# david-wb/tiny-diffusion

Hardware: AMD Instinct MI355X
Metric: train images/s (q_sample+fwd+MSE+bwd+allreduce+Adam), MNIST 28x28 UNet fp32; 1000-step sample latency in `sample` (higher is better)
Workload: dtype f32; 1 GPU; diffusion.py unconditional MNIST 28x28 UNet, fp32, train step, batch 256/GPU (BASELINE.json configs[1]); global_batch=256, per_gpu_batch=256, parallelism=dp1

## Files before the change

### include/tdx.h

```cpp
#ifndef TDX_H
#define TDX_H

#include <stddef.h>
#include <stdint.h>

#ifdef __cplusplus
extern "C" {
#endif

#define TDX_VERSION 400

#define TDX_E_BADARG (-1)
#define TDX_E_SHAPE (-2)
#define TDX_E_WORKSPACE (-3)
#define TDX_E_STATE (-4)

typedef void* tdx_stream_t;

int tdx_version(void);
const char* tdx_error_string(int code);


int tdx_q_sample(const float* x0, const float* noise, const int64_t* t,
                 const float* sqrt_ac, const float* sqrt_1mac, float* x_t,
// ... 155 lines not shown
                           int B, int H, int W, int cin, int cout, int flags,
                           const float* in_scale, const float* in_shift,
                           const float* out_scale, const float* out_shift,
                           float* scratch, size_t scratch_floats, tdx_stream_t stream);
size_t tdx_conv3x3_splitk_scratch_floats(int B, int H, int W, int cin, int cout);
int tdx_conv3x3_wino_ok(int B, int H, int W, int cin, int cout);
int tdx_pack_conv3x3_wino(const float* w_oihw, float* u_fwd, float* u_dgrad, int cout, int cin, tdx_stream_t stream);
int tdx_conv3x3_fwd_wino(const float* in, const float* u, const float* bias, float* out, int B, int H, int W,
                         int cin, int cout, int flags, const float* out_scale, const float* out_shift,
                         float* stats_partial, tdx_stream_t stream);
int tdx_conv3x3_fwd_wino_infer(const float* in, const float* u, const float* bias, float* out, int B, int H, int W,
                               int cin, int cout, const float* out_scale, const float* out_shift, float* scratch,
                               size_t scratch_floats, tdx_stream_t stream);
int tdx_conv3x3_train_algo(int B, int H, int W, int cin, int cout, int role);
int tdx_conv3x3_infer_algo(int B, int H, int W, int cin, int cout);
int tdx_conv3x3_wgrad_wino_splits(int B, int H, int W, int cin, int cout);
int tdx_conv3x3_wgrad_wino(const float* in, const float* dy, float* dw_slabs, int B, int H, int W, int cin, int cout,
                           tdx_stream_t stream);
int tdx_conv3x3_wino_stat_tiles(int B, int H, int W);
int tdx_conv3x3_wino_stat_tile_rows(int B, int H, int W);
int tdx_pack_conv3x3_tiled(const float* w_oihw, float* w_tiled, int cout, int cin, tdx_stream_t stream);
int tdx_conv3x3_fwd_infer(const float* in, const float* w_tiled, const float* bias, float* out, int B, int H, int W,
                          int cin, int cout, const float* out_scale, const float* out_shift, float* scratch,
                          size_t scratch_floats, tdx_stream_t stream);
size_t tdx_conv3x3_infer_scratch_floats(int B, int H, int W, int cin, int cout);
int tdx_conv3x3_fwd_train(const float* in, const float* wpk, const float* bias, float* out, int B, int H, int W,
                          int cin, int cout, int flags, float* stats_partial, float* scratch,
                          size_t scratch_floats, tdx_stream_t stream);
size_t tdx_conv3x3_train_scratch_floats(int B, int H, int W, int cin, int cout);
int tdx_conv3x3_stat_tiles(int B, int H, int W, int cin, int cout);
// ... 44 lines not shown
                    const float* save_rstd, const float* gamma,
                    float* dgamma, float* dbeta, float* dbias, float* scratch,
                    int training, tdx_stream_t stream);
size_t tdx_bn_relu_bwd_scratch_floats(int64_t rows, int C);

int tdx_maxpool2_ceil_fwd(const float* y, const float* scale, const float* shift, float* out,
                          int B, int H, int W, int C, tdx_stream_t stream);
int tdx_maxpool2_ceil_bwd(const float* y, const float* scale, const float* shift,
                          const float* g_out, const float* skip_grad, float* g_in,
                          int B, int H, int W, int C, tdx_stream_t stream);

int tdx_bilinear_ac_fwd(const float* in, const float* scale, const float* shift,
                        const float* addend, float* out,
                        int B, int Hi, int Wi, int Ho, int Wo, int C,
                        int out_cstride, int out_coff, tdx_stream_t stream);
int tdx_bilinear_ac_bwd(const float* g_out, float* g_in,
                        int B, int Hi, int Wi, int Ho, int Wo, int C,
                        int g_cstride, int g_coff, tdx_stream_t stream);


enum {
  TDX_P_TE0_W = 0, TDX_P_TE0_B, TDX_P_TE2_W, TDX_P_TE2_B,
  TDX_P_CLASS_EMB,
  TDX_P_INIT_W, TDX_P_INIT_B,
  TDX_P_UNIT0,
  TDX_P_FINAL_W = TDX_P_UNIT0 + 13 * 4, TDX_P_FINAL_B,
  TDX_P_TP1_W, TDX_P_TP1_B, TDX_P_TP2_W, TDX_P_TP2_B, TDX_P_TP3_W, TDX_P_TP3_B,
  TDX_P_COUNT
};
#define TDX_B_COUNT (13 * 3)
// ... 60 lines not shown
typedef struct tdx_unet tdx_unet;

int tdx_unet_create(tdx_unet** out, int max_batch, int num_classes);
enum { TDX_UNET_MNIST = 0, TDX_UNET_LAION = 1, TDX_UNET_LATENT_MLP = 2 };
int tdx_unet_create_ex(tdx_unet** out, int max_batch, int kind, int num_classes);
int tdx_unet_create_hw(tdx_unet** out, int max_batch, int kind, int num_classes, int hw);
int tdx_unet_create_full(tdx_unet** out, int max_batch, int kind, int num_classes, int hw, int time_dim);
typedef int (*tdx_allreduce_fn)(void* user, double* device_buffer, int n, tdx_stream_t stream);
int tdx_unet_set_bn_sync(tdx_unet* u, tdx_allreduce_fn fn, void* user, double* buffer);

int tdx_unet_set_streams(tdx_unet* u, int mode);

#define TDX_PREC_F32 0
#define TDX_PREC_BF16 1
int tdx_unet_set_precision(tdx_unet* u, int precision);
int tdx_unet_destroy(tdx_unet* u);
size_t tdx_unet_workspace_bytes(const tdx_unet* u, int batch, int mode);

int tdx_unet_forward(tdx_unet* u, const void* const* params, void* const* buffers,
                     const float* x, const int64_t* t, const void* cond, float* out,
                     void* workspace, size_t workspace_bytes, int batch, int mode,
                     tdx_stream_t stream);

int tdx_unet_backward_stages(void);
int tdx_unet_backward(tdx_unet* u, const void* const* params, void* const* grads,
                      const float* d_out, void* workspace, size_t workspace_bytes,
                      int batch, int stage_lo, int stage_hi, tdx_stream_t stream);
int tdx_unet_backward_join(tdx_unet* u, tdx_stream_t stream);
int tdx_unet_backward_mark(tdx_unet* u, int slot);
int tdx_unet_backward_wait_mark(tdx_unet* u, int slot, tdx_stream_t stream);
// ... 61 lines not shown
```

### tiny_diffusion_amd/_lib.py

```python
from __future__ import annotations

import contextlib
import ctypes as C
import os

import torch

from . import _build

_c_float_p = C.c_void_p
_c_i64_p = C.c_void_p
_ptr = C.c_void_p


class TdxError(RuntimeError):
    pass


def _load():
    path = _build.LIB
    if not os.path.exists(path):
        if os.environ.get("TDX_NO_AUTOBUILD"):
            raise TdxError(
                f"{path} not found: build it with `python -m tiny_diffusion_amd._build` "
# ... 85 lines not shown
    "tdx_conv3x3_shape_ok": (C.c_int, [C.c_int] * 5),
    "tdx_conv3x3_tile_shape": (C.c_int, [C.c_int] * 6),
    "tdx_conv3x3_wgrad": (C.c_int, [_ptr, _ptr, _ptr, C.c_int, C.c_int, C.c_int, C.c_int, C.c_int,
                                    C.c_int, _ptr, _ptr, _ptr]),
    "tdx_conv3x3_wgrad_reduce": (C.c_int, [_ptr, _ptr, C.c_int, C.c_int, C.c_int, _ptr]),
    "tdx_bn_finalize": (C.c_int, [_ptr, C.c_int, C.c_int, C.c_int64, C.c_int, _ptr, _ptr, _ptr, _ptr, _ptr,
                                  _ptr, _ptr, _ptr, _ptr, C.c_int, _ptr]),
    "tdx_bn_relu_bwd": (C.c_int, [_ptr, _ptr, C.c_int64, C.c_int, _ptr, _ptr, _ptr, _ptr, _ptr,
                                  _ptr, _ptr, _ptr, _ptr, C.c_int, _ptr]),
    "tdx_bn_relu_bwd_scratch_floats": (C.c_size_t, [C.c_int64, C.c_int]),
    "tdx_maxpool2_ceil_fwd": (C.c_int, [_ptr, _ptr, _ptr, _ptr, C.c_int, C.c_int, C.c_int, C.c_int, _ptr]),
    "tdx_maxpool2_ceil_bwd": (C.c_int, [_ptr, _ptr, _ptr, _ptr, _ptr, _ptr, C.c_int, C.c_int, C.c_int,
                                        C.c_int, _ptr]),
    "tdx_bilinear_ac_fwd": (C.c_int, [_ptr, _ptr, _ptr, _ptr, _ptr, C.c_int, C.c_int, C.c_int, C.c_int,
                                      C.c_int, C.c_int, C.c_int, C.c_int, _ptr]),
    "tdx_bilinear_ac_bwd": (C.c_int, [_ptr, _ptr, C.c_int, C.c_int, C.c_int, C.c_int, C.c_int, C.c_int,
                                      C.c_int, C.c_int, _ptr]),
    "tdx_adam_step_dev": (C.c_int, [_ptr, _ptr, _ptr, _ptr, C.c_int64, _ptr, C.c_float, C.c_float, C.c_float, _ptr]),
    "tdx_step_begin": (C.c_int, [_ptr, _ptr, _ptr, C.c_int, _ptr]),
    "tdx_step_begin_sched": (C.c_int, [_ptr, _ptr, _ptr, _ptr, C.c_int, _ptr]),
    "tdx_p_sample_step_sched": (C.c_int, [_ptr, _ptr, _ptr, _ptr, _ptr, _ptr, _ptr, C.c_int64, _ptr]),
    "tdx_p_sample_step_sched_philox": (C.c_int, [_ptr, _ptr, _ptr, _ptr, _ptr, _ptr, C.c_int64, C.c_uint64, _ptr]),
    "tdx_linear_fwd": (C.c_int, [_ptr, C.c_int, _ptr, _ptr, _ptr, C.c_int, C.c_int, C.c_int, C.c_int, C.c_int, _ptr]),
    "tdx_linear_bwd": (C.c_int, [_ptr, C.c_int, _ptr, C.c_int, _ptr, _ptr, C.c_int, _ptr, _ptr, C.c_int, C.c_int,
                                 C.c_int, _ptr]),
    "tdx_linear_fwd_prec": (C.c_int, [_ptr, C.c_int, _ptr, _ptr, _ptr, C.c_int, C.c_int, C.c_int, C.c_int, C.c_int, C.c_int,
                                      _ptr]),
    "tdx_linear_bwd_prec": (C.c_int, [_ptr, C.c_int, _ptr, C.c_int, _ptr, _ptr, C.c_int, _ptr, _ptr, C.c_int, C.c_int,
                                      C.c_int, C.c_int, _ptr]),
    "tdx_vae_workspace_floats": (C.c_size_t, [C.c_int, C.c_int]),
# ... 12 lines not shown
    "tdx_act_fwd": (C.c_int, [_ptr, _ptr, C.c_int64, C.c_int, _ptr]),
    "tdx_act_bwd": (C.c_int, [_ptr, _ptr, _ptr, C.c_int64, C.c_int, _ptr]),
    "tdx_dropout": (C.c_int, [_ptr, _ptr, C.c_int64, C.c_int, C.c_float, C.c_uint64, C.c_uint64, _ptr]),
    "tdx_add": (C.c_int, [_ptr, _ptr, _ptr, C.c_int64, C.c_int64, _ptr]),
    "tdx_embedding_fwd": (C.c_int, [_ptr, _ptr, _ptr, C.c_int, C.c_int, _ptr]),
    "tdx_embedding_bwd": (C.c_int, [_ptr, _ptr, _ptr, C.c_int, C.c_int, C.c_int, _ptr]),
    "tdx_transformer_train_workspace_floats": (C.c_size_t, [_ptr]),
    "tdx_transformer_loss_grads": (C.c_int, [_ptr] * 8 + [C.c_int, C.c_uint64, C.c_uint64, _ptr, C.c_float] + [_ptr] * 4),
    "tdx_unet_create": (C.c_int, [C.POINTER(_ptr), C.c_int, C.c_int]),
    "tdx_unet_create_ex": (C.c_int, [C.POINTER(_ptr), C.c_int, C.c_int, C.c_int]),
    "tdx_unet_create_hw": (C.c_int, [C.POINTER(_ptr), C.c_int, C.c_int, C.c_int, C.c_int]),
    "tdx_unet_create_full": (C.c_int, [C.POINTER(_ptr), C.c_int, C.c_int, C.c_int, C.c_int, C.c_int]),
    "tdx_unet_set_bn_sync": (C.c_int, [_ptr, _ptr, _ptr, _ptr]),
    "tdx_unet_set_streams": (C.c_int, [_ptr, C.c_int]),
    "tdx_unet_set_precision": (C.c_int, [_ptr, C.c_int]),
    "tdx_pack_conv3x3_bf16": (C.c_int, [_ptr, _ptr, _ptr, C.c_int, C.c_int, _ptr]),
    "tdx_conv3x3_bf16_stat_tile_rows": (C.c_int, []),
    "tdx_conv3x3_fwd_bf16": (C.c_int, [_ptr, _ptr, _ptr, _ptr, C.c_int, C.c_int, C.c_int, C.c_int, C.c_int,
                                       C.c_int, _ptr, _ptr, _ptr, _ptr, _ptr, _ptr]),
    "tdx_conv3x3_wgrad_bf16": (C.c_int, [_ptr, _ptr, _ptr, C.c_int, C.c_int, C.c_int, C.c_int, C.c_int,
                                         C.c_int, _ptr, _ptr, _ptr]),
    "tdx_unet_destroy": (C.c_int, [_ptr]),
    "tdx_unet_workspace_bytes": (C.c_size_t, [_ptr, C.c_int, C.c_int]),
    "tdx_unet_forward": (C.c_int, [_ptr, _ptr, _ptr, _ptr, _ptr, _ptr, _ptr, _ptr, C.c_size_t, C.c_int,
                                   C.c_int, _ptr]),
    "tdx_unet_backward_stages": (C.c_int, []),
    "tdx_unet_backward": (C.c_int, [_ptr, _ptr, _ptr, _ptr, _ptr, C.c_size_t, C.c_int, C.c_int, C.c_int,
                                    _ptr]),
    "tdx_unet_backward_join": (C.c_int, [_ptr, _ptr]),
    "tdx_unet_backward_mark": (C.c_int, [_ptr, C.c_int]),
# ... 97 lines not shown
    return value.value


@contextlib.contextmanager
def tuned(**knobs):
    old = [(key, tune_get(key)) for key in knobs]
    try:
        for key, value in knobs.items():
            check(lib.tdx_tune_set(key.encode(), int(value)), f"tdx_tune_set({key})")
        yield
    finally:
        for key, value in reversed(old):
            check(lib.tdx_tune_set(key.encode(), value), f"tdx_tune_set({key})")


def ptr(t):
    return None if t is None else t.data_ptr()


def stream_ptr(device=None):
    return torch.cuda.current_stream(device).cuda_stream
```

### tiny_diffusion_amd/csrc/conv3x3.hip

```cpp
#include "internal.h"

#define BK 32
#define BKP 36

#include "conv_shared.h"

template <int BM, int BN, int EPI>
__global__ void __launch_bounds__(256)
conv3x3_igemm_kernel(ConvArgs a) {
  constexpr int WGM = 2, WGN = 2;
  constexpr int WTM = BM / WGM, WTN = BN / WGN;
  constexpr int TM = WTM / 32, TN = WTN / 32;
  constexpr int AI = BM / 32, BI = BN / 32;
  static_assert(TM >= 1 && TN >= 1, "wave tile must hold a 32x32 MFMA tile");

  extern __shared__ __attribute__((aligned(16))) float smem[];
  float* As = smem;
  float* Bs = smem + 2 * BM * BKP;

  const int tid = threadIdx.x;
  const int lane = tid & 63, wave = tid >> 6;
  const int l31 = lane & 31, half = lane >> 5;
  const int wm = wave / WGN, wn = wave % WGN;
  const int xb = blockIdx.x / (8 * a.tilesN), xr = blockIdx.x % (8 * a.tilesN);
// ... 1237 lines not shown
  a.bias = bias; a.out = scratch; a.out_scale = out_scale; a.out_shift = out_shift;
  a.B = B; a.H = H; a.W = W; a.Cin = cin; a.Cout = cout; a.M = (int)M;
  bool pooled = false;
  const int rc = splitk_finish<EPI_BNRELU>(a, out, scratch, splits, to_stream(stream), defer, pool ? pool->pooled : nullptr, &pooled);
  if (pool && !pooled) pool->pooled = nullptr;
  return rc;
}

extern "C" int tdx_conv3x3_fwd_wino_infer(const float* in, const float* u, const float* bias, float* out, int B, int H,
                                         int W, int cin, int cout, const float* out_scale, const float* out_shift,
                                         float* scratch, size_t scratch_floats, tdx_stream_t stream) {
  return tdx_conv3x3_fwd_wino_infer_ex(in, u, bias, out, B, H, W, cin, cout, out_scale, out_shift, scratch, scratch_floats,
                                       stream, nullptr, nullptr);
}

extern "C" int tdx_conv3x3_fwd_infer(const float* in, const float* w_tiled, const float* bias, float* out, int B, int H,
                                     int W, int cin, int cout, const float* out_scale, const float* out_shift,
                                     float* scratch, size_t scratch_floats, tdx_stream_t stream) {
  return tdx_conv3x3_fwd_infer_ex(in, w_tiled, bias, out, B, H, W, cin, cout, out_scale, out_shift, scratch,
                                  scratch_floats, stream, nullptr, nullptr);
}

extern "C" size_t tdx_conv3x3_infer_scratch_floats(int B, int H, int W, int cin, int cout) {
  int per;
  const int64_t M = (int64_t)B * H * W;
  if (B <= 0 || H <= 0 || W <= 0 || cin % BK || cout % 64) return 0;
  const int s = plan_infer(M, cin, cout, &per, (size_t)-1);
  return s > 1 ? (size_t)s * M * cout : 0;
}

// ... 578 lines not shown
```

### tiny_diffusion_amd/csrc/spatial.hip

```cpp
#include "internal.h"
#include "io16.h"

__device__ static inline float4 bnrelu4(float4 v, const float4& sc, const float4& sh) {
  v.x = fmaxf(fmaf(v.x, sc.x, sh.x), 0.f);
  v.y = fmaxf(fmaf(v.y, sc.y, sh.y), 0.f);
  v.z = fmaxf(fmaf(v.z, sc.z, sh.z), 0.f);
  v.w = fmaxf(fmaf(v.w, sc.w, sh.w), 0.f);
  return v;
}

struct BnBwdOps {
  const void* y;
  const float* scale; const float* shift; const float* mean; const float* rstd;
  float* partial;
};
__device__ static inline void bnbwd_acc(const float4& g, const float4& y, const float4& sc, const float4& sh,
                                        const float4& mu, const float4& rs, float4& s1, float4& s2) {
#define ACC(k)                                                  \
  {                                                             \
    const float gz = fmaf(y.k, sc.k, sh.k) > 0.f ? g.k : 0.f;   \
    s1.k += gz;                                                 \
    s2.k += gz * ((y.k - mu.k) * rs.k);                         \
  }
  ACC(x) ACC(y) ACC(z) ACC(w)
// ... 322 lines not shown
                             hipStream_t st, int io16) {
  const bool deferred = a_defer && a_defer->splits > 0;
  if ((!a && !deferred) || (!b && Cb) || !out || Ca % 4 || Cb % 4 || Ca <= 0 || Cb < 0) return TDX_E_BADARG;
  if (deferred && (!a_defer->partial || !a_defer->scale || !a_defer->shift)) return TDX_E_BADARG;
  ResizeSrc A{deferred ? static_cast<const void*>(a_defer->partial) : a, nullptr, Ha, Wa, Ca, ac_scale(Ha, Ho), ac_scale(Wa, Wo),
              deferred ? a_defer->splits : 0, deferred ? a_defer->slab : 0, deferred ? a_defer->bias : nullptr,
              deferred ? a_defer->scale : nullptr, deferred ? a_defer->shift : nullptr};
  ResizeSrc Bs{b, b_addend, Cb ? Hb : 1, Cb ? Wb : 1, Cb, Cb ? ac_scale(Hb, Ho) : 0.f, Cb ? ac_scale(Wb, Wo) : 0.f,
               0, 0, nullptr, nullptr, nullptr};
  const int64_t n = (int64_t)B * Ho * Wo * ((Ca + Cb) / 4);
  TDX_IO_DISPATCH(io16, T, bilinear_pair_fwd_kernel<T><<<ew_grid(n), 256, 0, st>>>(A, Bs, (T*)out, B, Ho, Wo));
  TDX_CHECK_LAUNCH();
  return 0;
}

#define BIL_MAXC 8
__device__ static inline void axis_adjoint(int i, float scale, int n_in, int n_out, int& lo,
                                           float (&w)[BIL_MAXC]) {
  int hi;
  if (scale > 0.f) {
    lo = max(0, (int)floorf((float)(i - 1) / scale) - 1);
    hi = min(n_out - 1, (int)ceilf((float)(i + 1) / scale) + 1);
  } else {
    lo = 0;
    hi = n_out - 1;
  }
  if (hi - lo + 1 > BIL_MAXC) hi = lo + BIL_MAXC - 1;
#pragma unroll
  for (int k = 0; k < BIL_MAXC; ++k) {
    const int o = lo + k;
// ... 226 lines not shown
```

### tiny_diffusion_amd/csrc/unet.hip

```cpp
#include "internal.h"
#include <algorithm>
#include <cstdlib>
#include <mutex>
#include <new>
#include <string>
#include <vector>

namespace {

struct UnitDef {
  int cin, cout, hw;
  int in_bn;
  int cin_real;
};

struct NetSpec {
  int in_ch, hw0, out_hw;
  int x0_ch, x0_real;
  int overlap;
  int time_dim;
  int enc_hw[4];
  int dec_hw[3];
  int skip_ch[3];
  UnitDef units[13];
// ... 30 lines not shown
  return true;
}


inline size_t align64(size_t n) { return (n + 63) / 64 * 64; }

struct Layout {
  size_t x, t, y;
  size_t sin, pre, emb, tp[3];
  size_t x0, Y[13], ss[13];
  size_t A[13];
  size_t ep[3], cat[3], d1a;
  size_t stats;
  size_t ksplit, ksplit_floats;
  size_t G1, G2, G3, G4, GS[3], gtp[3], slabs, slabs2, bnscr, smallp, smallp2, timescr;
  size_t gbuf;
  size_t total;
};

Layout make_layout(const NetSpec& S, int B) {
  Layout L;
  size_t o = 0;
  auto take = [&](size_t n) { size_t r = o; o += align64(n); return r; };
  const size_t b = (size_t)B;
  const size_t px0 = (size_t)S.hw0 * S.hw0;
  L.x = take(b * px0 * S.in_ch); L.t = take(2 * b); L.y = take(std::max<size_t>(2 * b, b * S.time_dim));
  L.sin = take(b * S.time_dim); L.pre = take(b * S.time_dim); L.emb = take(b * S.time_dim);
  for (int k = 0; k < 3; ++k) L.tp[k] = take(b * S.skip_ch[k]);
  L.x0 = take(b * px0 * S.x0_ch);
  size_t stats = 0, slabs = 0, bnscr = 0, gbuf = 0, ksplit = 0;
  for (int u = 0; u < 13; ++u) {
    const UnitDef& d = S.units[u];
    L.Y[u] = take(b * d.hw * d.hw * d.cout);
    L.ss[u] = take(4 * (size_t)d.cout);
    L.A[u] = (u + 1 < 13 && S.units[u + 1].in_bn) ? take(b * d.hw * d.hw * d.cout) : 0;
    stats = std::max(stats, (size_t)tdx_conv3x3_stat_tiles(B, d.hw, d.hw, d.cin, d.cout) * 2 * d.cout);
    slabs = std::max(slabs, (size_t)std::max(std::max(tdx_conv3x3_wgrad_splits(B, d.hw, d.hw, d.cin, d.cout),
                                                      tdx_conv3x3_wgrad_splits_bf16(B, d.hw, d.hw, d.cin, d.cout)),
                                             tdx_conv3x3_wgrad_wino_splits(B, d.hw, d.hw, d.cin, d.cout)) *
                                9 * (size_t)d.cin * d.cout);
    ksplit = std::max(ksplit, std::max(tdx_conv3x3_train_scratch_floats(B, d.hw, d.hw, d.cin, d.cout),
                                       tdx_conv3x3_train_scratch_floats(B, d.hw, d.hw, d.cout, d.cin)));
    bnscr = std::max(bnscr, tdx_bn_relu_bwd_scratch_floats((int64_t)b * d.hw * d.hw, d.cout));
    gbuf = std::max(gbuf, b * d.hw * d.hw * (size_t)std::max(d.cin, d.cout));
  }
  for (int k = 0; k < 3; ++k) {
    const int hp = S.enc_hw[k + 1];
    L.ep[k] = take(b * hp * hp * S.skip_ch[k]);
  }
  for (int k = 0; k < 3; ++k) {
    const UnitDef& d = S.units[7 + 2 * k];
    L.cat[k] = take(b * d.hw * d.hw * d.cin);
  }
  L.d1a = take(b * S.out_hw * S.out_hw * 64);
  gbuf = std::max(gbuf, b * (size_t)S.out_hw * S.out_hw * 64);
  L.stats = take(stats);
  L.ksplit_floats = ksplit;
  L.ksplit = take(ksplit);
  L.gbuf = gbuf;
  L.G1 = take(gbuf); L.G2 = take(gbuf); L.G3 = take(gbuf); L.G4 = take(gbuf);
  for (int k = 0; k < 3; ++k) {
    L.GS[k] = take(b * S.enc_hw[k] * S.enc_hw[k] * S.skip_ch[k]);
    L.gtp[k] = take(b * S.skip_ch[k]);
  }
  L.slabs = take(slabs);
  L.slabs2 = take(slabs);
  L.bnscr = take(bnscr);
  L.smallp = take((size_t)tdx_small_conv_wgrad_blocks(B, S.hw0, S.hw0) * tdx_small_conv_partial_width());
  L.smallp2 = take((size_t)tdx_small_conv_wgrad_blocks(B, S.hw0, S.hw0) * tdx_small_conv_partial_width());
  L.timescr = take(3 * b * S.time_dim);
  L.total = o;
  return L;
}

}

struct PlanHandles {
  hipStream_t side, side2, half;
  hipEvent_t ev[81];
};

// ... 181 lines not shown
extern "C" int tdx_unet_set_bn_sync(tdx_unet* u, tdx_allreduce_fn fn, void* user, double* buffer) {
  if (!u || (fn && !buffer)) return TDX_E_BADARG;
  if (!u->spec) return fn ? TDX_E_SHAPE : 0;
  u->bn_sync = fn;
  u->bn_sync_user = user;
  u->bn_sync_buf = buffer;
  return 0;
}

extern "C" int tdx_unet_set_streams(tdx_unet* u, int mode) {
  if (!u || mode < -1 || mode > 2) return TDX_E_BADARG;
  u->use_streams = mode < 0 ? (u->spec ? u->spec->overlap : 0) : mode;
  return 0;
}

extern "C" int tdx_unet_set_precision(tdx_unet* u, int precision) {
  if (!u || (precision != TDX_PREC_F32 && precision != TDX_PREC_BF16)) return TDX_E_BADARG;
  if (!u->spec) { u->precision = precision; return 0; }
  if (precision != u->precision) u->packed = false;
  u->precision = precision;
  u->io16 = precision == TDX_PREC_BF16 && g_knobs.bf16_storage ? 1 : 0;
  return 0;
}

extern "C" int tdx_unet_destroy(tdx_unet* u) {
  if (!u) return TDX_E_BADARG;
  recycle_handles(u->handles);
  (void)hipFree(u->wpack);
  if (u->upack) (void)hipFree(u->upack);
  (void)hipFree(u->infer_ss);
// ... 270 lines not shown
    const float* src[3] = {x, reinterpret_cast<const float*>(t), reinterpret_cast<const float*>(labels)};
    float* dst[3] = {ws + L.x, ws + L.t, ws + L.y};
    const size_t cnt[3] = {nx, 2 * (size_t)B, labels ? 2 * (size_t)B : 0};
    RC(tdx_copy_segments(src, dst, cnt, 3, st));
  }

  hipStream_t tst = st;
  if (!infer && u->side2 != st) {
    TDX_HIP(hipEventRecord(u->ev_fork, st));
    TDX_HIP(hipStreamWaitEvent(u->side2, u->ev_fork, 0));
    tst = u->side2;
  }
  if (!(infer && u->skip_time_path))
    RC(tdx_time_embed_fwd(u->kind, t, labels, cond_emb, P, ws + L.sin, ws + L.pre, ws + L.emb, ws + L.tp[0],
                          ws + L.tp[1], ws + L.tp[2], B, tst, S.time_dim));
  RC(tdx_initial_conv_fwd(x, P[TDX_P_INIT_W], P[TDX_P_INIT_B], ws + L.x0, B, S.hw0, S.hw0, S.in_ch,
                          S.x0_real, st, io16));

  auto sc = [&](int i) -> const float* { return infer ? nullptr : ws + L.ss[i]; };
  auto sh = [&](int i) -> const float* { return infer ? nullptr : ws + L.ss[i] + S.units[i].cout; };

  auto finalize_bn = [&](int i, int tiles, int tile_rows, int64_t count) -> int {
    const UnitDef& d = S.units[i];
    float* ss = ws + L.ss[i];
    if (training && u->bn_sync) {
      RC(tdx_bn_moments(ws + L.stats, tiles, tile_rows, count, d.cout, u->bn_sync_buf, st));
      RC(u->bn_sync(u->bn_sync_user, u->bn_sync_buf, 2 * d.cout + 1, stream));
      return tdx_bn_finalize_moments(u->bn_sync_buf, d.cout, P[TDX_P_UNIT0 + 4 * i + 2], P[TDX_P_UNIT0 + 4 * i + 3],
                                     (float*)buffers[3 * i], (float*)buffers[3 * i + 1], (int64_t*)buffers[3 * i + 2],
                                     ss, ss + d.cout, ss + 2 * d.cout, ss + 3 * d.cout, st);
// ... 32 lines not shown
    if (infer) {
      const float* iss = u->infer_ss + u->iss_off[i];
      if (u->wino_f[i] && tdx_conv3x3_infer_algo(B, d.hw, d.hw, d.cin, d.cout))
        return tdx_conv3x3_fwd_wino_infer_ex(in, u->upack + u->uf_off[i], bias, Y, B, d.hw, d.hw, d.cin, d.cout, iss,
                                             iss + d.cout, ws + L.G1, 2 * L.gbuf, stream, defer, pool);
      if (u->wf_tiled)
        return tdx_conv3x3_fwd_infer_ex(in, wf, bias, Y, B, d.hw, d.hw, d.cin, d.cout, iss, iss + d.cout, ws + L.G1,
                                        2 * L.gbuf, stream, defer, pool);
      return tdx_conv3x3_fwd_splitk_fused(in, wf, bias, Y, B, d.hw, d.hw, d.cin, d.cout, TDX_CONV_OUT_BNRELU, iss,
                                          iss + d.cout, ws + L.G1, 2 * L.gbuf, stream, defer, pool);
    }
    const bool bn_on_load = d.in_bn && !u->materialize;
    if (d.in_bn && u->materialize) in = ws + L.A[i - 1];
    int flags = (bn_on_load ? TDX_CONV_IN_BNRELU : 0) | (training ? TDX_CONV_OUT_STATS : 0);
    if (u->wino_f[i] && !bn_on_load) {
      RC(tdx_conv3x3_fwd_wino(in, u->upack + u->uf_off[i], bias, Y, B, d.hw, d.hw, d.cin, d.cout,
                              training ? TDX_CONV_OUT_STATS : 0, nullptr, nullptr, ws + L.stats, stream));
      RC(finalize_bn(i, tdx_conv3x3_wino_stat_tiles(B, d.hw, d.hw), tdx_conv3x3_wino_stat_tile_rows(B, d.hw, d.hw),
                     (int64_t)B * d.hw * d.hw));
      if (u->materialize && i + 1 < 13 && S.units[i + 1].in_bn)
        RC(tdx_bn_relu_apply(Y, ws + L.A[i], (int64_t)B * d.hw * d.hw, d.cout, ss, ss + d.cout, st));
      return 0;
    }
    if (bn_on_load)
      RC(tdx_conv3x3_fwd(in, wf, bias, Y, B, d.hw, d.hw, d.cin, d.cout, flags, sc(i - 1), sh(i - 1), nullptr, nullptr,
                         ws + L.stats, stream));
    else
      RC(tdx_conv3x3_fwd_train(in, wf, bias, Y, B, d.hw, d.hw, d.cin, d.cout, flags, ws + L.stats, ws + L.ksplit,
                               L.ksplit_floats, stream));
    const int tiles = tdx_conv3x3_stat_tiles(B, d.hw, d.hw, d.cin, d.cout);
    RC(finalize_bn(i, tiles, tdx_conv3x3_stat_tile_rows(B, d.hw, d.hw, d.cin, d.cout), (int64_t)B * d.hw * d.hw));
    if (u->materialize && i + 1 < 13 && S.units[i + 1].in_bn)
      RC(tdx_bn_relu_apply(Y, ws + L.A[i], (int64_t)B * d.hw * d.hw, d.cout, ss, ss + d.cout, st));
    return 0;
  };

  RC(run_unit(0, ws + L.x0));
  if (!infer) RC(pack_tail(u, params, stream));
  for (int k = 0; k < 3; ++k) {
    const int ua = 2 * k, ub = 2 * k + 1;
    if (k == 1 && !infer) TDX_HIP(hipStreamWaitEvent(st, u->ev_pack, 0));
    if (k > 0) RC(run_unit(ua, ws + L.ep[k - 1]));
    TdxPoolFuse pf{infer && !bf16 && (g_knobs.sample_fuse & 2) ? ws + L.ep[k] : nullptr};
    RC(run_unit(ub, ws + L.Y[ua], nullptr, pf.pooled ? &pf : nullptr));
    if (!infer) {
      const int kd = 2 - k, ud = 7 + 2 * kd;
      const UnitDef& dd = S.units[ud];
      const int c_up = S.units[kd == 0 ? 6 : 6 + 2 * kd].cout;
      TDX_HIP(hipEventRecord(u->ev_s2_fork[k], st));
      TDX_HIP(hipStreamWaitEvent(u->side2, u->ev_s2_fork[k], 0));
      RC(tdx_bilinear_ac_fwd_t(ws + L.Y[ub], sc(ub), sh(ub), ws + L.tp[k], ws + L.cat[kd], B, S.enc_hw[k],
                               S.enc_hw[k], dd.hw, dd.hw, S.skip_ch[k], dd.cin, c_up, io16,
                               reinterpret_cast<tdx_stream_t>(u->side2)));
      TDX_HIP(hipEventRecord(u->ev_s2_done[k], u->side2));
    }
    if (!pf.pooled)
      RC(tdx_maxpool2_ceil_fwd_t(ws + L.Y[ub], sc(ub), sh(ub), ws + L.ep[k], B, S.enc_hw[k], S.enc_hw[k],
                                 S.skip_ch[k], io16, stream));
  }
  const bool defer_ok = infer && !bf16 && (g_knobs.sample_fuse & 1);
  TdxSplitDefer dfr{};
  RC(run_unit(6, ws + L.ep[2], defer_ok ? &dfr : nullptr));
  for (int k = 0; k < 3; ++k) {
    const int ua = 7 + 2 * k, ub = 8 + 2 * k;
    const int prev = k == 0 ? 6 : 6 + 2 * k;
    const int skip_u = 5 - 2 * k;
    const int skip_k = 2 - k;
    const UnitDef& da = S.units[ua];
    const UnitDef& dp = S.units[prev];
    const int hw = da.hw, c_up = dp.cout, c_skip = S.skip_ch[skip_k];
    if (infer) {
      RC(tdx_bilinear_pair_fwd_ex(ws + L.Y[prev], &dfr, dp.hw, dp.hw, c_up, ws + L.Y[skip_u], ws + L.tp[skip_k],
                                  S.enc_hw[skip_k], S.enc_hw[skip_k], c_skip, ws + L.cat[k], B, hw, hw, st, io16));
      dfr = TdxSplitDefer{};
    } else {
      RC(tdx_bilinear_ac_fwd_t(ws + L.Y[prev], sc(prev), sh(prev), nullptr, ws + L.cat[k], B, dp.hw, dp.hw, hw, hw,
                               c_up, da.cin, 0, io16, stream));
      TDX_HIP(hipStreamWaitEvent(st, u->ev_s2_done[skip_k], 0));
    }
    RC(run_unit(ua, ws + L.cat[k]));
    RC(run_unit(ub, ws + L.Y[ua], defer_ok ? &dfr : nullptr));
  }
  if (dfr.splits > 0)
    RC(tdx_bilinear_pair_fwd_ex(nullptr, &dfr, S.dec_hw[2], S.dec_hw[2], 64, nullptr, nullptr, 0, 0, 0, ws + L.d1a, B,
                                S.out_hw, S.out_hw, st));
  else
    RC(tdx_bilinear_ac_fwd_t(ws + L.Y[12], sc(12), sh(12), nullptr, ws + L.d1a, B, S.dec_hw[2], S.dec_hw[2],
                             S.out_hw, S.out_hw, 64, 64, 0, io16, stream));
  if (infer && ps.x)
    RC(tdx_final_conv_fwd_psample(ws + L.d1a, P[TDX_P_FINAL_W], P[TDX_P_FINAL_B], out, B, S.out_hw, S.out_hw, S.in_ch,
                                  ps, st, io16));
  else
    RC(tdx_final_conv_fwd(ws + L.d1a, P[TDX_P_FINAL_W], P[TDX_P_FINAL_B], out, B, S.out_hw, S.out_hw, S.in_ch, st, io16));
// ... 508 lines not shown
```

Measured before the change: 27600 images/s.

## Fuse encoder maxpool with skip resize and add split-K Winograd forward

Adds a kernel that loads each encoder output band into LDS once, applies BN+ReLU, and writes both the 2x2 maxpool and the bilinear skip upsample (plus time-embedding addend). This replaces the separate pool kernel and the side-stream resize, along with their event synchronisation. It also adds a split-K Winograd forward path for small-spatial, wide-channel layers that have too few workgroups to fill the CUs. That path reduces the partial slabs in a kernel that also emits BN statistics. Both are on by default, but they serialise the skip resize onto the main stream and need extra scratch traffic for the split-K partials.

```diff
diff --git a/include/tdx.h b/include/tdx.h
--- a/include/tdx.h
+++ b/include/tdx.h
@@ -193,6 +193,13 @@
                                size_t scratch_floats, tdx_stream_t stream);
 int tdx_conv3x3_train_algo(int B, int H, int W, int cin, int cout, int role);
 int tdx_conv3x3_infer_algo(int B, int H, int W, int cin, int cout);
+int tdx_conv3x3_fwd_wino_splitk(const float* in, const float* u, const float* bias, float* out, int B, int H, int W,
+                                int cin, int cout, int splits, float* scratch, size_t scratch_floats,
+                                float* stats_partial, tdx_stream_t stream);
+int tdx_conv3x3_wino_splitk_stat_tile_rows(int cout);
+int tdx_conv3x3_wino_splitk_stat_tiles(int B, int H, int W, int cout);
+int tdx_conv3x3_wino_train_splits(int B, int H, int W, int cin, int cout, int cus);
+
 int tdx_conv3x3_wgrad_wino_splits(int B, int H, int W, int cin, int cout);
 int tdx_conv3x3_wgrad_wino(const float* in, const float* dy, float* dw_slabs, int B, int H, int W, int cin, int cout,
                            tdx_stream_t stream);
@@ -267,6 +274,9 @@
                         const float* addend, float* out,
                         int B, int Hi, int Wi, int Ho, int Wo, int C,
                         int out_cstride, int out_coff, tdx_stream_t stream);
+int tdx_pool_skip_fwd(const void* y, const float* scale, const float* shift, const float* addend,
+                      void* pooled, void* out, int B, int H, int W, int Ho, int Wo, int C,
+                      int out_cstride, int out_coff, int io16, tdx_stream_t stream);
 int tdx_bilinear_ac_bwd(const float* g_out, float* g_in,
                         int B, int Hi, int Wi, int Ho, int Wo, int C,
                         int g_cstride, int g_coff, tdx_stream_t stream);
@@ -357,6 +367,10 @@
 #define TDX_PREC_F32 0
 #define TDX_PREC_BF16 1
 int tdx_unet_set_precision(tdx_unet* u, int precision);
+#define TDX_FUSE_POOL_SKIP 1
+#define TDX_FUSE_FWD_SPLITK 2
+int tdx_forward_fusion_set(int mask);
+int tdx_forward_fusion_get(void);
 int tdx_unet_destroy(tdx_unet* u);
 size_t tdx_unet_workspace_bytes(const tdx_unet* u, int batch, int mode);
 
diff --git a/tiny_diffusion_amd/_lib.py b/tiny_diffusion_amd/_lib.py
--- a/tiny_diffusion_amd/_lib.py
+++ b/tiny_diffusion_amd/_lib.py
@@ -123,6 +123,13 @@
                                         C.c_int, _ptr]),
     "tdx_bilinear_ac_fwd": (C.c_int, [_ptr, _ptr, _ptr, _ptr, _ptr, C.c_int, C.c_int, C.c_int, C.c_int,
                                       C.c_int, C.c_int, C.c_int, C.c_int, _ptr]),
+    "tdx_conv3x3_fwd_wino_splitk": (C.c_int, [_ptr, _ptr, _ptr, _ptr, C.c_int, C.c_int, C.c_int, C.c_int, C.c_int,
+                                              C.c_int, _ptr, C.c_size_t, _ptr, _ptr]),
+    "tdx_conv3x3_wino_splitk_stat_tile_rows": (C.c_int, [C.c_int]),
+    "tdx_conv3x3_wino_splitk_stat_tiles": (C.c_int, [C.c_int, C.c_int, C.c_int, C.c_int]),
+    "tdx_conv3x3_wino_train_splits": (C.c_int, [C.c_int, C.c_int, C.c_int, C.c_int, C.c_int, C.c_int]),
+    "tdx_pool_skip_fwd": (C.c_int, [_ptr, _ptr, _ptr, _ptr, _ptr, _ptr, C.c_int, C.c_int, C.c_int, C.c_int,
+                                    C.c_int, C.c_int, C.c_int, C.c_int, C.c_int, _ptr]),
     "tdx_bilinear_ac_bwd": (C.c_int, [_ptr, _ptr, C.c_int, C.c_int, C.c_int, C.c_int, C.c_int, C.c_int,
                                       C.c_int, C.c_int, _ptr]),
     "tdx_adam_step_dev": (C.c_int, [_ptr, _ptr, _ptr, _ptr, C.c_int64, _ptr, C.c_float, C.c_float, C.c_float, _ptr]),
@@ -165,6 +172,8 @@
     "tdx_unet_set_bn_sync": (C.c_int, [_ptr, _ptr, _ptr, _ptr]),
     "tdx_unet_set_streams": (C.c_int, [_ptr, C.c_int]),
     "tdx_unet_set_precision": (C.c_int, [_ptr, C.c_int]),
+    "tdx_forward_fusion_set": (C.c_int, [C.c_int]),
+    "tdx_forward_fusion_get": (C.c_int, []),
     "tdx_pack_conv3x3_bf16": (C.c_int, [_ptr, _ptr, _ptr, C.c_int, C.c_int, _ptr]),
     "tdx_conv3x3_bf16_stat_tile_rows": (C.c_int, []),
     "tdx_conv3x3_fwd_bf16": (C.c_int, [_ptr, _ptr, _ptr, _ptr, C.c_int, C.c_int, C.c_int, C.c_int, C.c_int,
@@ -292,6 +301,16 @@
             check(lib.tdx_tune_set(key.encode(), value), f"tdx_tune_set({key})")
 
 
+@contextlib.contextmanager
+def forward_fusion(mask: int):
+    old = lib.tdx_forward_fusion_get()
+    check(lib.tdx_forward_fusion_set(int(mask)), "tdx_forward_fusion_set")
+    try:
+        yield
+    finally:
+        check(lib.tdx_forward_fusion_set(old), "tdx_forward_fusion_set")
+
+
 def ptr(t):
     return None if t is None else t.data_ptr()
 
diff --git a/tiny_diffusion_amd/csrc/conv3x3.hip b/tiny_diffusion_amd/csrc/conv3x3.hip
--- a/tiny_diffusion_amd/csrc/conv3x3.hip
+++ b/tiny_diffusion_amd/csrc/conv3x3.hip
@@ -1275,6 +1275,102 @@
                                        stream, nullptr, nullptr);
 }
 
+#define SKS_ROWS 4
+__global__ void __launch_bounds__(256)
+splitk_reduce_stats_kernel(const float* __restrict__ partial, int splits, size_t slab, int M, int cout,
+                           const float* __restrict__ bias, float* __restrict__ out, float* __restrict__ stats) {
+  __shared__ float4 red[256];
+  __shared__ float4 tot[256];
+  const int c4n = cout / 4, col = threadIdx.x % c4n, rg = threadIdx.x / c4n, rgroups = 256 / c4n;
+  const int tile_rows = SKS_ROWS * rgroups, row0 = blockIdx.x * tile_rows, nrows = min(tile_rows, M - row0);
+  const float4 bv = bias ? *reinterpret_cast<const float4*>(bias + col * 4) : make_float4(0.f, 0.f, 0.f, 0.f);
+  float4 v[SKS_ROWS];
+  float4 s = make_float4(0.f, 0.f, 0.f, 0.f);
+#pragma unroll
+  for (int r = 0; r < SKS_ROWS; ++r) {
+    const int lr = r * rgroups + rg;
+    v[r] = bv;
+    if (lr < nrows) {
+      const size_t off = (size_t)(row0 + lr) * cout + col * 4;
+      for (int sp = 0; sp < splits; ++sp) {
+        const float4 t = *reinterpret_cast<const float4*>(partial + (size_t)sp * slab + off);
+        v[r].x += t.x; v[r].y += t.y; v[r].z += t.z; v[r].w += t.w;
+      }
+      *reinterpret_cast<float4*>(out + off) = v[r];
+      s.x += v[r].x; s.y += v[r].y; s.z += v[r].z; s.w += v[r].w;
+    }
+  }
+  if (!stats) return;
+  red[threadIdx.x] = s;
+  __syncthreads();
+  if (rg == 0) {
+    float4 t = red[col];
+    for (int k = 1; k < rgroups; ++k) {
+      const float4 o = red[k * c4n + col];
+      t.x += o.x; t.y += o.y; t.z += o.z; t.w += o.w;
+    }
+    tot[col] = t;
+    *reinterpret_cast<float4*>(stats + ((size_t)blockIdx.x * 2 + 0) * cout + col * 4) = t;
+  }
+  __syncthreads();
+  const float inv = 1.0f / (float)nrows;
+  const float4 t = tot[col];
+  const float4 mu = make_float4(t.x * inv, t.y * inv, t.z * inv, t.w * inv);
+  float4 q = make_float4(0.f, 0.f, 0.f, 0.f);
+#pragma unroll
+  for (int r = 0; r < SKS_ROWS; ++r)
+    if (r * rgroups + rg < nrows) {
+      const float dx = v[r].x - mu.x, dy = v[r].y - mu.y, dz = v[r].z - mu.z, dw = v[r].w - mu.w;
+      q.x += dx * dx; q.y += dy * dy; q.z += dz * dz; q.w += dw * dw;
+    }
+  red[threadIdx.x] = q;
+  __syncthreads();
+  if (rg == 0) {
+    float4 m2 = red[col];
+    for (int k = 1; k < rgroups; ++k) {
+      const float4 o = red[k * c4n + col];
+      m2.x += o.x; m2.y += o.y; m2.z += o.z; m2.w += o.w;
+    }
+    *reinterpret_cast<float4*>(stats + ((size_t)blockIdx.x * 2 + 1) * cout + col * 4) = m2;
+  }
+}
+
+static bool sks_width_ok(int cout) { return cout > 0 && cout % 4 == 0 && cout <= 1024 && 256 % (cout / 4) == 0; }
+extern "C" int tdx_conv3x3_wino_splitk_stat_tile_rows(int cout) {
+  return sks_width_ok(cout) ? SKS_ROWS * (256 / (cout / 4)) : 0;
+}
+extern "C" int tdx_conv3x3_wino_splitk_stat_tiles(int B, int H, int W, int cout) {
+  const int rows = tdx_conv3x3_wino_splitk_stat_tile_rows(cout);
+  return rows ? (int)cdiv((int64_t)B * H * W, rows) : 0;
+}
+
+extern "C" int tdx_conv3x3_wino_train_splits(int B, int H, int W, int cin, int cout, int cus) {
+  if (cus <= 0 || !tdx_conv3x3_wino_ok(B, H, W, cin, cout) || !sks_width_ok(cout)) return 1;
+  const int64_t wgs = (int64_t)tdx_conv3x3_wino_stat_tiles(B, H, W) * (cout / 64);
+  if (wgs > cus / 2) return 1;
+  const int ns = cin / 8;
+  const int s = (int)std::min<int64_t>(cus / wgs, ns / 8);
+  if (s < 2) return 1;
+  const int per = (ns + s - 1) / s;
+  return (ns + per - 1) / per;
+}
+
+extern "C" int tdx_conv3x3_fwd_wino_splitk(const float* in, const float* u, const float* bias, float* out, int B, int H,
+                                          int W, int cin, int cout, int splits, float* scratch, size_t scratch_floats,
+                                          float* stats_partial, tdx_stream_t stream) {
+  if (!in || !u || !out || !scratch || splits < 2) return TDX_E_BADARG;
+  if (!tdx_conv3x3_wino_ok(B, H, W, cin, cout) || !sks_width_ok(cout)) return TDX_E_SHAPE;
+  const int ns = cin / 8, per = (ns + splits - 1) / splits;
+  if ((ns + per - 1) / per != splits) return TDX_E_BADARG;
+  const size_t slab = (size_t)B * H * W * cout;
+  if (scratch_floats < (size_t)splits * slab) return TDX_E_WORKSPACE;
+  RC_(tdx_conv3x3_wino_launch(in, u, nullptr, scratch, B, H, W, cin, cout, 0, nullptr, nullptr, nullptr, splits, per, stream));
+  splitk_reduce_stats_kernel<<<tdx_conv3x3_wino_splitk_stat_tiles(B, H, W, cout), 256, 0, to_stream(stream)>>>(
+      scratch, splits, slab, B * H * W, cout, bias, out, stats_partial);
+  TDX_CHECK_LAUNCH();
+  return 0;
+}
+
 extern "C" int tdx_conv3x3_fwd_infer(const float* in, const float* w_tiled, const float* bias, float* out, int B, int H,
                                      int W, int cin, int cout, const float* out_scale, const float* out_shift,
                                      float* scratch, size_t scratch_floats, tdx_stream_t stream) {
diff --git a/tiny_diffusion_amd/csrc/spatial.hip b/tiny_diffusion_amd/csrc/spatial.hip
--- a/tiny_diffusion_amd/csrc/spatial.hip
+++ b/tiny_diffusion_amd/csrc/spatial.hip
@@ -1,3 +1,4 @@
+#include <climits>
 #include "internal.h"
 #include "io16.h"
 
@@ -360,6 +361,153 @@
   return 0;
 }
 
+#define POOL_SKIP_LDS_BYTES (40 * 1024)
+
+__device__ static inline int first_dst_with_i0_ge(int r, float scale, int n_in, int n_out) {
+  if (r <= 0) return 0;
+  if (r > n_in - 1) return n_out;
+  int o = scale > 0.f ? (int)fminf((float)r / scale, (float)n_out) : n_out;
+  o = min(max(o, 0), n_out);
+  while (o > 0 && axis_tap(o - 1, scale, n_in).i0 >= r) --o;
+  while (o < n_out && axis_tap(o, scale, n_in).i0 < r) ++o;
+  return o;
+}
+
+template <typename T>
+__global__ void __launch_bounds__(256)
+pool_skip_fwd_kernel(const T* __restrict__ y, const float* __restrict__ scale, const float* __restrict__ shift,
+                     const float* __restrict__ addend, T* __restrict__ pooled, T* __restrict__ out, int H, int W,
+                     int Ho, int Wo, int C, int ocs, int ocoff, float sch, float scw, int bands, int band_rows,
+                     int chunk) {
+  extern __shared__ float4 tile[];
+  const int b = blockIdx.x / bands, band = blockIdx.x - b * bands;
+  const int r0 = band * band_rows, r1 = min(r0 + band_rows, H);
+  const int c0 = blockIdx.y * chunk, c4n = min(chunk, C - c0) / 4;
+  const int Hp = (H + 1) / 2, Wp = (W + 1) / 2;
+  const int p0 = r0 / 2, p1 = (r1 + 1) / 2;
+  const int o0 = first_dst_with_i0_ge(r0, sch, H, Ho), o1 = first_dst_with_i0_ge(r1, sch, H, Ho);
+  const int n_ld = (min(r1 + 1, H) - r0) * W * c4n;
+  const bool fixed = 256 % c4n == 0;
+  const int step = fixed ? 256 / c4n : 256;
+  const int px0 = threadIdx.x / c4n;
+  int c = (threadIdx.x % c4n) * 4;
+  float4 sc = *reinterpret_cast<const float4*>(scale + c0 + c), sh = *reinterpret_cast<const float4*>(shift + c0 + c);
+  const T* base = y + ((int64_t)b * H + r0) * W * C + c0;
+  for (int j0 = threadIdx.x; j0 < n_ld; j0 += 4 * 256) {
+    float4 v[4];
+#pragma unroll
+    for (int k = 0; k < 4; ++k) {
+      const int j = j0 + k * 256;
+      if (j < n_ld) v[k] = fixed ? ld4(base + (int64_t)(px0 + (j >> 8) * step) * C + c)
+                                 : ld4(base + (int64_t)(j / c4n) * C + (j % c4n) * 4);
+    }
+#pragma unroll
+    for (int k = 0; k < 4; ++k) {
+      const int j = j0 + k * 256;
+      if (j < n_ld) {
+        if (!fixed) {
+          c = (j % c4n) * 4;
+          sc = *reinterpret_cast<const float4*>(scale + c0 + c);
+          sh = *reinterpret_cast<const float4*>(shift + c0 + c);
+        }
+        tile[j] = bnrelu4(v[k], sc, sh);
+      }
+    }
+  }
+  __syncthreads();
+  const float* adp = addend ? addend + (int64_t)b * C + c0 : nullptr;
+  float4 ad = make_float4(0.f, 0.f, 0.f, 0.f);
+  if (fixed && adp) ad = *reinterpret_cast<const float4*>(adp + (threadIdx.x % c4n) * 4);
+
+  auto pool_item = [&](int cq, int oh, int ow) {
+    float4 m = make_float4(-INFINITY, -INFINITY, -INFINITY, -INFINITY);
+#pragma unroll
+    for (int dh = 0; dh < 2; ++dh)
+#pragma unroll
+      for (int dw = 0; dw < 2; ++dw) {
+        const int ih = 2 * oh + dh, iw = 2 * ow + dw;
+        if (ih < H && iw < W) {
+          const float4 v = tile[((ih - r0) * W + iw) * c4n + cq];
+          m.x = fmaxf(m.x, v.x); m.y = fmaxf(m.y, v.y);
+          m.z = fmaxf(m.z, v.z); m.w = fmaxf(m.w, v.w);
+        }
+      }
+    st4(pooled + (((int64_t)b * Hp + oh) * Wp + ow) * C + c0 + cq * 4, m);
+  };
+  auto resize_item = [&](int cq, int oh, int ow) {
+    const AxisTap th = axis_tap(oh, sch, H), tw = axis_tap(ow, scw, W);
+    auto ld = [&](int h, int w) {
+      float4 v = tile[((h - r0) * W + w) * c4n + cq];
+      v.x += ad.x; v.y += ad.y; v.z += ad.z; v.w += ad.w;
+      return v;
+    };
+    const float4 v00 = ld(th.i0, tw.i0), v01 = ld(th.i0, tw.i1);
+    const float4 v10 = ld(th.i1, tw.i0), v11 = ld(th.i1, tw.i1);
+    float4 o;
+#define LERP(k)                                          \
+    {                                                    \
+      const float top = tw.l0 * v00.k + tw.l1 * v01.k;   \
+      const float bot = tw.l0 * v10.k + tw.l1 * v11.k;   \
+      o.k = th.l0 * top + th.l1 * bot;                   \
+    }
+    LERP(x) LERP(y) LERP(z) LERP(w)
+#undef LERP
+    st4(out + (((int64_t)b * Ho + oh) * Wo + ow) * ocs + ocoff + c0 + cq * 4, o);
+  };
+  if (fixed) {
+    const int cq = threadIdx.x % c4n, px = px0;
+    int oh = p0 + px / Wp, ow = px % Wp;
+    while (oh < p1) {
+      pool_item(cq, oh, ow);
+      ow += step;
+      while (ow >= Wp) { ow -= Wp; ++oh; }
+    }
+    oh = o0 + px / Wo; ow = px % Wo;
+    while (oh < o1) {
+      resize_item(cq, oh, ow);
+      ow += step;
+      while (ow >= Wo) { ow -= Wo; ++oh; }
+    }
+  } else {
+    const int n_pool = (p1 - p0) * Wp * c4n, n_all = n_pool + (o1 - o0) * Wo * c4n;
+    for (int j = threadIdx.x; j < n_all; j += 256) {
+      const bool pool = j < n_pool;
+      int p = pool ? j : j - n_pool;
+      const int cq = p % c4n;
+      p /= c4n;
+      if (pool) {
+        pool_item(cq, p0 + p / Wp, p % Wp);
+      } else {
+        if (adp) ad = *reinterpret_cast<const float4*>(adp + cq * 4);
+        resize_item(cq, o0 + p / Wo, p % Wo);
+      }
+    }
+  }
+}
+
+extern "C" int tdx_pool_skip_fwd(const void* y, const float* scale, const float* shift, const float* addend,
+                                 void* pooled, void* out, int B, int H, int W, int Ho, int Wo, int C, int out_cstride,
+                                 int out_coff, int io16, tdx_stream_t stream) {
+  if (!y || !scale || !shift || !pooled || !out || B <= 0 || H <= 0 || W <= 0 || Ho <= 0 || Wo <= 0 || C <= 0)
+    return TDX_E_BADARG;
+  if (C % 4 || out_cstride % 4 || out_coff % 4 || out_coff + C > out_cstride) return TDX_E_SHAPE;
+  int band_rows = 4, chunk = C < 64 ? C : 64;
+  auto lds_bytes = [&]() { return (int64_t)(band_rows + 1) * W * chunk * (int64_t)sizeof(float); };
+  while (lds_bytes() > POOL_SKIP_LDS_BYTES && chunk > 4) chunk = chunk > 8 ? chunk / 2 / 4 * 4 : 4;
+  if (lds_bytes() > POOL_SKIP_LDS_BYTES) band_rows = 2;
+  if (lds_bytes() > POOL_SKIP_LDS_BYTES) return TDX_E_SHAPE;
+  const int bands = (H + band_rows - 1) / band_rows, chunks = (C + chunk - 1) / chunk;
+  if ((int64_t)B * bands > INT_MAX || chunks > 65535 ||
+      ((int64_t)band_rows * ((W + 1) / 2) + (int64_t)Ho * Wo) * (chunk / 4) > INT_MAX)
+    return TDX_E_SHAPE;
+  const dim3 grid(B * bands, chunks);
+  TDX_IO_DISPATCH(io16, T, pool_skip_fwd_kernel<T><<<grid, 256, (size_t)lds_bytes(), to_stream(stream)>>>(
+      (const T*)y, scale, shift, addend, (T*)pooled, (T*)out, H, W, Ho, Wo, C, out_cstride, out_coff,
+      ac_scale(H, Ho), ac_scale(W, Wo), bands, band_rows, chunk));
+  TDX_CHECK_LAUNCH();
+  return 0;
+}
+
 #define BIL_MAXC 8
 __device__ static inline void axis_adjoint(int i, float scale, int n_in, int n_out, int& lo,
                                            float (&w)[BIL_MAXC]) {
diff --git a/tiny_diffusion_amd/csrc/unet.hip b/tiny_diffusion_amd/csrc/unet.hip
--- a/tiny_diffusion_amd/csrc/unet.hip
+++ b/tiny_diffusion_amd/csrc/unet.hip
@@ -68,6 +68,7 @@
   size_t stats;
   size_t ksplit, ksplit_floats;
   size_t G1, G2, G3, G4, GS[3], gtp[3], slabs, slabs2, bnscr, smallp, smallp2, timescr;
+  size_t slab_region;
   size_t gbuf;
   size_t total;
 };
@@ -89,6 +90,7 @@
     L.ss[u] = take(4 * (size_t)d.cout);
     L.A[u] = (u + 1 < 13 && S.units[u + 1].in_bn) ? take(b * d.hw * d.hw * d.cout) : 0;
     stats = std::max(stats, (size_t)tdx_conv3x3_stat_tiles(B, d.hw, d.hw, d.cin, d.cout) * 2 * d.cout);
+    stats = std::max(stats, (size_t)tdx_conv3x3_wino_splitk_stat_tiles(B, d.hw, d.hw, d.cout) * 2 * d.cout);
     slabs = std::max(slabs, (size_t)std::max(std::max(tdx_conv3x3_wgrad_splits(B, d.hw, d.hw, d.cin, d.cout),
                                                       tdx_conv3x3_wgrad_splits_bf16(B, d.hw, d.hw, d.cin, d.cout)),
                                              tdx_conv3x3_wgrad_wino_splits(B, d.hw, d.hw, d.cin, d.cout)) *
@@ -119,6 +121,7 @@
   }
   L.slabs = take(slabs);
   L.slabs2 = take(slabs);
+  L.slab_region = o - L.slabs;
   L.bnscr = take(bnscr);
   L.smallp = take((size_t)tdx_small_conv_wgrad_blocks(B, S.hw0, S.hw0) * tdx_small_conv_partial_width());
   L.smallp2 = take((size_t)tdx_small_conv_wgrad_blocks(B, S.hw0, S.hw0) * tdx_small_conv_partial_width());
@@ -330,6 +333,25 @@
   return 0;
 }
 
+static int g_forward_fusion = TDX_FUSE_POOL_SKIP | TDX_FUSE_FWD_SPLITK;
+extern "C" int tdx_forward_fusion_set(int mask) {
+  if (mask & ~(TDX_FUSE_POOL_SKIP | TDX_FUSE_FWD_SPLITK)) return TDX_E_BADARG;
+  g_forward_fusion = mask;
+  return 0;
+}
+extern "C" int tdx_forward_fusion_get(void) { return g_forward_fusion; }
+
+static int device_cus() {
+  static int cus = 0;
+  if (!cus) {
+    int dev = 0, n = 0;
+    if (hipGetDevice(&dev) == hipSuccess &&
+        hipDeviceGetAttribute(&n, hipDeviceAttributeMultiprocessorCount, dev) == hipSuccess && n > 0)
+      cus = n;
+  }
+  return cus;
+}
+
 extern "C" int tdx_unet_set_precision(tdx_unet* u, int precision) {
   if (!u || (precision != TDX_PREC_F32 && precision != TDX_PREC_BF16)) return TDX_E_BADARG;
   if (!u->spec) { u->precision = precision; return 0; }
@@ -630,6 +652,8 @@
   if (!(infer && u->skip_time_path))
     RC(tdx_time_embed_fwd(u->kind, t, labels, cond_emb, P, ws + L.sin, ws + L.pre, ws + L.emb, ws + L.tp[0],
                           ws + L.tp[1], ws + L.tp[2], B, tst, S.time_dim));
+  const bool pool_skip = !infer && (g_forward_fusion & TDX_FUSE_POOL_SKIP);
+  if (pool_skip && tst != st) TDX_HIP(hipEventRecord(u->ev_s2_done[0], tst));
   RC(tdx_initial_conv_fwd(x, P[TDX_P_INIT_W], P[TDX_P_INIT_B], ws + L.x0, B, S.hw0, S.hw0, S.in_ch,
                           S.x0_real, st, io16));
 
@@ -692,10 +716,19 @@
     if (d.in_bn && u->materialize) in = ws + L.A[i - 1];
     int flags = (bn_on_load ? TDX_CONV_IN_BNRELU : 0) | (training ? TDX_CONV_OUT_STATS : 0);
     if (u->wino_f[i] && !bn_on_load) {
-      RC(tdx_conv3x3_fwd_wino(in, u->upack + u->uf_off[i], bias, Y, B, d.hw, d.hw, d.cin, d.cout,
-                              training ? TDX_CONV_OUT_STATS : 0, nullptr, nullptr, ws + L.stats, stream));
-      RC(finalize_bn(i, tdx_conv3x3_wino_stat_tiles(B, d.hw, d.hw), tdx_conv3x3_wino_stat_tile_rows(B, d.hw, d.hw),
-                     (int64_t)B * d.hw * d.hw));
+      const int splits = (g_forward_fusion & TDX_FUSE_FWD_SPLITK)
+                             ? tdx_conv3x3_wino_train_splits(B, d.hw, d.hw, d.cin, d.cout, device_cus()) : 1;
+      if (splits > 1 && (size_t)splits * B * d.hw * d.hw * d.cout <= L.slab_region) {
+        RC(tdx_conv3x3_fwd_wino_splitk(in, u->upack + u->uf_off[i], bias, Y, B, d.hw, d.hw, d.cin, d.cout, splits,
+                                       ws + L.slabs, L.slab_region, training ? ws + L.stats : nullptr, stream));
+        RC(finalize_bn(i, tdx_conv3x3_wino_splitk_stat_tiles(B, d.hw, d.hw, d.cout),
+                       tdx_conv3x3_wino_splitk_stat_tile_rows(d.cout), (int64_t)B * d.hw * d.hw));
+      } else {
+        RC(tdx_conv3x3_fwd_wino(in, u->upack + u->uf_off[i], bias, Y, B, d.hw, d.hw, d.cin, d.cout,
+                                training ? TDX_CONV_OUT_STATS : 0, nullptr, nullptr, ws + L.stats, stream));
+        RC(finalize_bn(i, tdx_conv3x3_wino_stat_tiles(B, d.hw, d.hw), tdx_conv3x3_wino_stat_tile_rows(B, d.hw, d.hw),
+                       (int64_t)B * d.hw * d.hw));
+      }
       if (u->materialize && i + 1 < 13 && S.units[i + 1].in_bn)
         RC(tdx_bn_relu_apply(Y, ws + L.A[i], (int64_t)B * d.hw * d.hw, d.cout, ss, ss + d.cout, st));
       return 0;
@@ -721,10 +754,16 @@
     if (k > 0) RC(run_unit(ua, ws + L.ep[k - 1]));
     TdxPoolFuse pf{infer && !bf16 && (g_knobs.sample_fuse & 2) ? ws + L.ep[k] : nullptr};
     RC(run_unit(ub, ws + L.Y[ua], nullptr, pf.pooled ? &pf : nullptr));
+    const int kd = 2 - k, ud = 7 + 2 * kd;
+    const UnitDef& dd = S.units[ud];
+    const int c_up = S.units[kd == 0 ? 6 : 6 + 2 * kd].cout;
+    if (pool_skip) {
+      if (k == 0 && tst != st) TDX_HIP(hipStreamWaitEvent(st, u->ev_s2_done[0], 0));
+      RC(tdx_pool_skip_fwd(ws + L.Y[ub], sc(ub), sh(ub), ws + L.tp[k], ws + L.ep[k], ws + L.cat[kd], B, S.enc_hw[k],
+                           S.enc_hw[k], dd.hw, dd.hw, S.skip_ch[k], dd.cin, c_up, io16, stream));
+      continue;
+    }
     if (!infer) {
-      const int kd = 2 - k, ud = 7 + 2 * kd;
-      const UnitDef& dd = S.units[ud];
-      const int c_up = S.units[kd == 0 ? 6 : 6 + 2 * kd].cout;
       TDX_HIP(hipEventRecord(u->ev_s2_fork[k], st));
       TDX_HIP(hipStreamWaitEvent(u->side2, u->ev_s2_fork[k], 0));
       RC(tdx_bilinear_ac_fwd_t(ws + L.Y[ub], sc(ub), sh(ub), ws + L.tp[k], ws + L.cat[kd], B, S.enc_hw[k],
@@ -754,7 +793,7 @@
     } else {
       RC(tdx_bilinear_ac_fwd_t(ws + L.Y[prev], sc(prev), sh(prev), nullptr, ws + L.cat[k], B, dp.hw, dp.hw, hw, hw,
                                c_up, da.cin, 0, io16, stream));
-      TDX_HIP(hipStreamWaitEvent(st, u->ev_s2_done[skip_k], 0));
+      if (!pool_skip) TDX_HIP(hipStreamWaitEvent(st, u->ev_s2_done[skip_k], 0));
     }
     RC(run_unit(ua, ws + L.cat[k]));
     RC(run_unit(ub, ws + L.Y[ua], defer_ok ? &dfr : nullptr));
```

New measurement: 27830 images/s (median of 6 runs). About the same (+0.8%).
